# lucidrains/transfusion-pytorch

Measured on NVIDIA H100. Metric: train tokens/sec (text+latent) at d=512 L=8 seq=1024, higher is better.
Workload: dtype bf16

## Files before the change

transfusion_pytorch_b200/csrc/attention_sm90.cu:

```cuda
#include "sm90_ptx.cuh"
#include "common.cuh"
#include "gemm_sm90.cuh"
#include "../../include/tfx_b200.h"

namespace tfx {

int num_sms();

constexpr int FA_BM = 128, FA_BN = 128;
constexpr int FA_THREADS = 256;
constexpr int FA_SMEM = 16384 * 5 + 1024  + 256 ;
constexpr float FA_YMAX = 0.75f;

#define FA_C0 9.9999722832e-01f
#define FA_C1 -3.3323076483e-01f
#define FA_C2 1.3226091649e-01f
#define FA_C3 -4.9280448379e-02f
#define FA_C4 1.2318833231e-02f

__global__ void attn_fast_params_k(const float* __restrict__ gq, const float* __restrict__ gk, int n, float scale, float cap, float* __restrict__ params) {
  const int lane = threadIdx.x;
  float a = 0.f, b = 0.f;
  for (int i = lane; i < n; i += 32) { a = fmaxf(a, fabsf(gq[i] + 1.f)); b = fmaxf(b, fabsf(gk[i] + 1.f)); }
  a = warp_max(a); b = warp_max(b);
  if (lane == 0) {
    const float xmax = 1.01f * (float)n * a * b * scale;
    const float ymax = xmax / cap;
    params[0] = (ymax <= FA_YMAX && isfinite(ymax)) ? 1.f : 0.f;
    params[1] = xmax;
  }
}

__device__ __forceinline__ float ex2_approx(float x) { float y; asm("ex2.approx.ftz.f32 %0, %1;" : "=f"(y) : "f"(x)); return y; }

struct FaPoly {
  float a0, a1, a2, a3, a4;
  __device__ __forceinline__ FaPoly(float scale, float cap) {
    const float k1 = scale / cap, KL = cap * 1.4426950408889634f, k2 = k1 * k1;
    a0 = KL * k1 * FA_C0; a1 = KL * k1 * k2 * FA_C1; a2 = KL * k1 * k2 * k2 * FA_C2; a3 = KL * k1 * k2 * k2 * k2 * FA_C3; a4 = KL * k1 * k2 * k2 * k2 * k2 * FA_C4;
  }
  __device__ __forceinline__ float operator()(float x) const {
    const float X = x * x;
    float g = fmaf(a4, X, a3);
    g = fmaf(g, X, a2);
    g = fmaf(g, X, a1);
    g = fmaf(g, X, a0);
    return x * g;
  }
};

__global__ void __launch_bounds__(FA_THREADS, 2)
attn_fwd_tc_k(const __grid_constant__ CUtensorMap tmQ, const __grid_constant__ CUtensorMap tmK, const __grid_constant__ CUtensorMap tmV,
              const float* __restrict__ gates, int H, const int* __restrict__ kv_limit, const int* __restrict__ tile_q0, const int* __restrict__ tile_qend,
              const int* __restrict__ tile_kv0, const int* __restrict__ tile_kvend, __nv_bfloat16* __restrict__ o, long long ld_o, float* __restrict__ lse,
              int M, float scale, float cap, const float* __restrict__ fast) {
  if (fast[0] == 0.f) return;
  extern __shared__ uint8_t fa_smem_raw[];
  uint8_t* smem = reinterpret_cast<uint8_t*>((reinterpret_cast<uintptr_t>(fa_smem_raw) + 1023) & ~uintptr_t(1023));
  uint8_t* sQ = smem;
  uint8_t* sK = smem + 16384;
  uint8_t* sV = smem + 49152;
  uint64_t* bars = reinterpret_cast<uint64_t*>(smem + 81920);
  uint64_t *q_full = bars, *kv_full = bars + 1;

  const int tile = gridDim.x - 1 - blockIdx.x;
  const int head = blockIdx.y;
  const int tid = threadIdx.x, warp = tid >> 5, lane = tid & 31;
  const int cwg = warp >> 2, w4 = warp & 3, g = lane >> 2, t = lane & 3;
  const int q0 = tile_q0[tile], q_end = tile_qend[tile], kv0 = tile_kv0[tile], kv_end = tile_kvend[tile];
  const int n_kv = (kv_end - kv0 + FA_BN - 1) / FA_BN;

  if (tid == 0) {
    tma_prefetch_desc(&tmQ); tma_prefetch_desc(&tmK); tma_prefetch_desc(&tmV);
    mbar_init(q_full, 1); mbar_init(&kv_full[0], 1); mbar_init(&kv_full[1], 1);
    mbar_fence_init();
  }
  __syncthreads();
  if (tid == 0) {
    mbar_expect_tx(q_full, 16384);
    tma_load_2d(&tmQ, q_full, sQ, head * 64, q0);
    for (int j = 0; j < 2 && j < n_kv; ++j) {
      mbar_expect_tx(&kv_full[j], 32768);
      tma_load_2d(&tmK, &kv_full[j], sK + j * 16384, head * 64, kv0 + j * FA_BN);
      tma_load_2d(&tmV, &kv_full[j], sV + j * 16384, head * 64, kv0 + j * FA_BN);
    }
  }

  const int row_a = q0 + cwg * 64 + w4 * 16 + g, row_b = row_a + 8;
  const int lim_a = row_a < q_end ? kv_limit[row_a] : -1;
  const int lim_b = row_b < q_end ? kv_limit[row_b] : -1;
  const FaPoly poly(scale, cap);
  const float m2 = fast[1] * 1.4426950408889634f;
  float oacc[32];
#pragma unroll
  for (int i = 0; i < 32; ++i) oacc[i] = 0.f;
  float l_a = 0.f, l_b = 0.f;
  const uint32_t aQ = smem_u32(sQ) + cwg * 8192;
  mbar_wait(q_full, 0);

  for (int j = 0; j < n_kv; ++j) {
    const int b = j & 1;
    mbar_wait(&kv_full[b], (j >> 1) & 1);
    const uint32_t aK = smem_u32(sK + b * 16384), aV = smem_u32(sV + b * 16384);
    float s[64];
    wgmma_fence();
#pragma unroll
    for (int k = 0; k < 4; ++k) wgmma_m64n128_ss<0, 0>(s, wgmma_desc_sw128(aQ + k * 32, 16, 1024), wgmma_desc_sw128(aK + k * 32, 16, 1024), k > 0 ? 1u : 0u);
    wgmma_commit();
    wgmma_wait<0>();
    wgmma_reg_fence(s);
    const int key0 = kv0 + j * FA_BN;
    uint32_t pf[8][4];
#pragma unroll
    for (int n8 = 0; n8 < 16; ++n8) {
      const int key = key0 + n8 * 8 + 2 * t;
      float p0 = ex2_approx(poly(s[4 * n8]) - m2), p1 = ex2_approx(poly(s[4 * n8 + 1]) - m2);
      float p2 = ex2_approx(poly(s[4 * n8 + 2]) - m2), p3 = ex2_approx(poly(s[4 * n8 + 3]) - m2);
      p0 = key <= lim_a ? p0 : 0.f; p1 = key + 1 <= lim_a ? p1 : 0.f;
      p2 = key <= lim_b ? p2 : 0.f; p3 = key + 1 <= lim_b ? p3 : 0.f;
      l_a += p0 + p1; l_b += p2 + p3;
      pf[n8 >> 1][(n8 & 1) * 2] = pack_bf16(p0, p1);
      pf[n8 >> 1][(n8 & 1) * 2 + 1] = pack_bf16(p2, p3);
    }
    wgmma_reg_fence(oacc);
    wgmma_fence();
#pragma unroll
    for (int kk = 0; kk < 8; ++kk) wgmma_m64n64_rs<1>(oacc, pf[kk], wgmma_desc_sw128(aV + kk * 2048, 8192, 1024), 1u);
    wgmma_commit();
    wgmma_wait<0>();
    wgmma_reg_fence(oacc);
    __syncthreads();
    if (tid == 0 && j + 2 < n_kv) {
      mbar_expect_tx(&kv_full[b], 32768);
      tma_load_2d(&tmK, &kv_full[b], sK + b * 16384, head * 64, kv0 + (j + 2) * FA_BN);
      tma_load_2d(&tmV, &kv_full[b], sV + b * 16384, head * 64, kv0 + (j + 2) * FA_BN);
    }
  }
  l_a += __shfl_xor_sync(0xffffffffu, l_a, 1); l_a += __shfl_xor_sync(0xffffffffu, l_a, 2);
  l_b += __shfl_xor_sync(0xffffffffu, l_b, 1); l_b += __shfl_xor_sync(0xffffffffu, l_b, 2);
  float ga = l_a > 0.f ? 1.f / l_a : 0.f, gb = l_b > 0.f ? 1.f / l_b : 0.f;
  if (gates) {
    if (row_a < q_end) ga *= 1.f / (1.f + __expf(-gates[(long long)row_a * H + head]));
    if (row_b < q_end) gb *= 1.f / (1.f + __expf(-gates[(long long)row_b * H + head]));
  }
  if (row_a < q_end) {
    __nv_bfloat16* dst = o + (long long)row_a * ld_o + head * 64 + 2 * t;
#pragma unroll
    for (int n8 = 0; n8 < 8; ++n8) *reinterpret_cast<uint32_t*>(dst + n8 * 8) = pack_bf16(oacc[4 * n8] * ga, oacc[4 * n8 + 1] * ga);
    if (t == 0 && lse) lse[(long long)head * M + row_a] = fast[1] + logf(l_a);
  }
  if (row_b < q_end) {
    __nv_bfloat16* dst = o + (long long)row_b * ld_o + head * 64 + 2 * t;
#pragma unroll
    for (int n8 = 0; n8 < 8; ++n8) *reinterpret_cast<uint32_t*>(dst + n8 * 8) = pack_bf16(oacc[4 * n8 + 2] * gb, oacc[4 * n8 + 3] * gb);
    if (t == 0 && lse) lse[(long long)head * M + row_b] = fast[1] + logf(l_b);
  }
}


constexpr int FB_BQ = 64;
constexpr int FB_THREADS = 256;
constexpr int FB_SMEM = 16384 * 2  + 8192 * 4  + 16384  + 1024 + 256;

__global__ void __launch_bounds__(FB_THREADS, 1)
attn_bwd_tc_k(const __grid_constant__ CUtensorMap tmQ, const __grid_constant__ CUtensorMap tmK, const __grid_constant__ CUtensorMap tmV,
              const __grid_constant__ CUtensorMap tmDO,
              const float* __restrict__ lse, const float* __restrict__ dsum, const int* __restrict__ kv_limit,
              const int* __restrict__ kt_kv0, const int* __restrict__ kt_kvend, const int* __restrict__ kt_q0, const int* __restrict__ kt_qend,
              const int* __restrict__ kt_order, float* __restrict__ dq,
              float* __restrict__ dk, __nv_bfloat16* __restrict__ dv, long long ld_dv, int M, int H, float scale, float cap, const float* __restrict__ fast) {
  if (fast[0] == 0.f) return;
  extern __shared__ uint8_t fb_smem_raw[];
  uint8_t* smem = reinterpret_cast<uint8_t*>((reinterpret_cast<uintptr_t>(fb_smem_raw) + 1023) & ~uintptr_t(1023));
  uint8_t* sK = smem;
  uint8_t* sV = smem + 16384;
  uint8_t* sQ = smem + 32768;
  uint8_t* sDO = smem + 49152;
  uint8_t* sDS = smem + 65536;
  uint64_t* bars = reinterpret_cast<uint64_t*>(smem + 81920);
  uint64_t *kv_full = bars, *qdo_full = bars + 1;

  const int idx = blockIdx.x;
  const int tt = idx / H;
  const int tile = kt_order ? kt_order[tt] : tt;
  const int head = idx - tt * H;
  const int kv0 = kt_kv0[tile], kv_end = kt_kvend[tile], q_begin = kt_q0[tile], q_end = kt_qend[tile];
  const int n_q = (q_end - q_begin + FB_BQ - 1) / FB_BQ;
  const int tid = threadIdx.x, warp = tid >> 5, lane = tid & 31;
  const int cwg = warp >> 2, w4 = warp & 3, g = lane >> 2, t = lane & 3;
  const long long HI = (long long)H * 64;

  if (tid == 0) {
    tma_prefetch_desc(&tmQ); tma_prefetch_desc(&tmK); tma_prefetch_desc(&tmV); tma_prefetch_desc(&tmDO);
    mbar_init(kv_full, 1); mbar_init(&qdo_full[0], 1); mbar_init(&qdo_full[1], 1);
    mbar_fence_init();
  }
  __syncthreads();
  if (tid == 0) {
    mbar_expect_tx(kv_full, 32768);
    tma_load_2d(&tmK, kv_full, sK, head * 64, kv0);
    tma_load_2d(&tmV, kv_full, sV, head * 64, kv0);
    for (int i = 0; i < 2 && i < n_q; ++i) {
      mbar_expect_tx(&qdo_full[i], 16384);
      tma_load_2d(&tmQ, &qdo_full[i], sQ + i * 8192, head * 64, q_begin + i * FB_BQ);
      tma_load_2d(&tmDO, &qdo_full[i], sDO + i * 8192, head * 64, q_begin + i * FB_BQ);
    }
  }

  const FaPoly poly(scale, cap);
  const float KL = cap * 1.4426950408889634f;
  const float oms_c = -scale / (KL * KL);
  const int key_a = kv0 + cwg * 64 + w4 * 16 + g, key_b = key_a + 8;
  const float* lse_h = lse + (long long)head * M;
  const float* ds_h = dsum + (long long)head * M;
  float dvacc[32], dkacc[32];
#pragma unroll
  for (int i = 0; i < 32; ++i) { dvacc[i] = 0.f; dkacc[i] = 0.f; }
  const uint32_t aK = smem_u32(sK) + cwg * 8192, aV = smem_u32(sV) + cwg * 8192, aDS = smem_u32(sDS) + cwg * 8192;
  const int ds_row0 = cwg * 64 + w4 * 16 + g;
  mbar_wait(kv_full, 0);

  for (int i = 0; i < n_q; ++i) {
    const int b = i & 1;
    const int qb = q_begin + i * FB_BQ;
    mbar_wait(&qdo_full[b], (i >> 1) & 1);
    const uint32_t aQ = smem_u32(sQ + b * 8192), aDO = smem_u32(sDO + b * 8192);
    float sacc[32], pacc[32];
    wgmma_fence();
#pragma unroll
    for (int k = 0; k < 4; ++k) wgmma_m64n64_ss<0, 0>(sacc, wgmma_desc_sw128(aK + k * 32, 16, 1024), wgmma_desc_sw128(aQ + k * 32, 16, 1024), k > 0 ? 1u : 0u);
#pragma unroll
    for (int k = 0; k < 4; ++k) wgmma_m64n64_ss<0, 0>(pacc, wgmma_desc_sw128(aV + k * 32, 16, 1024), wgmma_desc_sw128(aDO + k * 32, 16, 1024), k > 0 ? 1u : 0u);
    wgmma_commit();
    wgmma_wait<0>();
    wgmma_reg_fence(sacc);
    wgmma_reg_fence(pacc);
    uint32_t pf[4][4], dsf[4][4];
#pragma unroll
    for (int n8 = 0; n8 < 8; ++n8) {
      float pv[4], dsv[4];
#pragma unroll
      for (int c = 0; c < 2; ++c) {
        const int qr = qb + n8 * 8 + 2 * t + c;
        const bool ok = qr < q_end;
        const int lim = ok ? kv_limit[qr] : -1;
        const float lse2 = ok ? lse_h[qr] * 1.4426950408889634f : 0.f;
        const float Dq = ok ? ds_h[qr] : 0.f;
#pragma unroll
        for (int r = 0; r < 2; ++r) {
          const int e = 4 * n8 + 2 * r + c;
          const float e2 = poly(sacc[e]);
          float p = ex2_approx(e2 - lse2);
          p = ((r == 0 ? key_a : key_b) <= lim) ? p : 0.f;
          pv[2 * r + c] = p;
          dsv[2 * r + c] = p * (pacc[e] - Dq) * fmaf(e2 * e2, oms_c, scale);
        }
      }
      pf[n8 >> 1][(n8 & 1) * 2] = pack_bf16(pv[0], pv[1]);
      pf[n8 >> 1][(n8 & 1) * 2 + 1] = pack_bf16(pv[2], pv[3]);
      dsf[n8 >> 1][(n8 & 1) * 2] = pack_bf16(dsv[0], dsv[1]);
      dsf[n8 >> 1][(n8 & 1) * 2 + 1] = pack_bf16(dsv[2], dsv[3]);
    }
    named_bar_sync(1 + cwg, 128);
#pragma unroll
    for (int n8 = 0; n8 < 8; ++n8) {
      const int r0 = ds_row0, r1 = ds_row0 + 8;
      *reinterpret_cast<uint32_t*>(sDS + r0 * 128 + ((n8 ^ (r0 & 7)) << 4) + t * 4) = dsf[n8 >> 1][(n8 & 1) * 2];
      *reinterpret_cast<uint32_t*>(sDS + r1 * 128 + ((n8 ^ (r1 & 7)) << 4) + t * 4) = dsf[n8 >> 1][(n8 & 1) * 2 + 1];
    }
    fence_proxy_async_smem();
    named_bar_sync(1 + cwg, 128);
    float qacc[32];
    wgmma_reg_fence(dvacc);
    wgmma_reg_fence(dkacc);
    wgmma_fence();
#pragma unroll
    for (int kk = 0; kk < 4; ++kk) wgmma_m64n64_rs<1>(dvacc, pf[kk], wgmma_desc_sw128(aDO + kk * 2048, 8192, 1024), 1u);
#pragma unroll
    for (int kk = 0; kk < 4; ++kk) wgmma_m64n64_rs<1>(dkacc, dsf[kk], wgmma_desc_sw128(aQ + kk * 2048, 8192, 1024), 1u);
#pragma unroll
    for (int kk = 0; kk < 4; ++kk) wgmma_m64n64_ss<1, 1>(qacc, wgmma_desc_sw128(aDS + kk * 2048, 8192, 1024), wgmma_desc_sw128(aK + kk * 2048, 8192, 1024), kk > 0 ? 1u : 0u);
    wgmma_commit();
    wgmma_wait<0>();
    wgmma_reg_fence(dvacc);
    wgmma_reg_fence(dkacc);
    wgmma_reg_fence(qacc);
    {
      const int r_a = qb + w4 * 16 + g, r_b = r_a + 8;
#pragma unroll
      for (int n8 = 0; n8 < 8; ++n8) {
        if (r_a < q_end) {
          float* d = dq + (long long)r_a * HI + head * 64 + n8 * 8 + 2 * t;
          asm volatile("red.global.add.v2.f32 [%0], {%1, %2};" ::"l"(d), "f"(qacc[4 * n8]), "f"(qacc[4 * n8 + 1]) : "memory");
        }
        if (r_b < q_end) {
          float* d = dq + (long long)r_b * HI + head * 64 + n8 * 8 + 2 * t;
          asm volatile("red.global.add.v2.f32 [%0], {%1, %2};" ::"l"(d), "f"(qacc[4 * n8 + 2]), "f"(qacc[4 * n8 + 3]) : "memory");
        }
      }
    }
    __syncthreads();
    if (tid == 0 && i + 2 < n_q) {
      mbar_expect_tx(&qdo_full[b], 16384);
      tma_load_2d(&tmQ, &qdo_full[b], sQ + b * 8192, head * 64, q_begin + (i + 2) * FB_BQ);
      tma_load_2d(&tmDO, &qdo_full[b], sDO + b * 8192, head * 64, q_begin + (i + 2) * FB_BQ);
    }
  }
#pragma unroll
  for (int n8 = 0; n8 < 8; ++n8) {
    if (key_a < kv_end) {
      *reinterpret_cast<float2*>(dk + (long long)key_a * HI + head * 64 + n8 * 8 + 2 * t) = make_float2(dkacc[4 * n8], dkacc[4 * n8 + 1]);
      *reinterpret_cast<uint32_t*>(dv + (long long)key_a * ld_dv + head * 64 + n8 * 8 + 2 * t) = pack_bf16(dvacc[4 * n8], dvacc[4 * n8 + 1]);
    }
    if (key_b < kv_end) {
      *reinterpret_cast<float2*>(dk + (long long)key_b * HI + head * 64 + n8 * 8 + 2 * t) = make_float2(dkacc[4 * n8 + 2], dkacc[4 * n8 + 3]);
      *reinterpret_cast<uint32_t*>(dv + (long long)key_b * ld_dv + head * 64 + n8 * 8 + 2 * t) = pack_bf16(dvacc[4 * n8 + 2], dvacc[4 * n8 + 3]);
    }
  }
}

}

using namespace tfx;
#define ST(s) reinterpret_cast<cudaStream_t>(s)

extern "C" {

int tfx_attn_fast_params(const float* q_gamma, const float* k_gamma, int dim_head, float scale, float softcap, float* params, void* stream) {
  TFX_REQUIRE(dim_head > 0 && softcap > 0.f, "attn_fast_params: bad arguments");
  attn_fast_params_k<<<1, 32, 0, ST(stream)>>>(q_gamma, k_gamma, dim_head, scale, softcap, params);
  return check_launch("attn_fast_params");
}

int tfx_attn_fwd_tc(const void* q, const void* k, const void* v, long long ld_q, long long ld_k, long long ld_v, const float* gates, int H,
                    const int* kv_limit, const int* tile_q0, const int* tile_qend, const int* tile_kv0, const int* tile_kvend, int n_tiles,
                    void* o, long long ld_o, float* lse, int M, int M_kv, float scale, float softcap, const float* fast_params, void* stream) {
  if (n_tiles <= 0) return 0;
  if (M_kv <= 0) M_kv = M;
  TFX_REQUIRE(fast_params != nullptr, "attn_fwd_tc: fast_params (from tfx_attn_fast_params) is required");
  TFX_REQUIRE(ld_q % 8 == 0 && ld_k % 8 == 0 && ld_v % 8 == 0 && ld_o % 8 == 0, "attn_fwd_tc: row pitches must be multiples of 8 bf16");
  CUtensorMap tq, tk, tv;
  int rc;
  if ((rc = make_tmap_bf16(&tq, q, (long long)H * 64, M, ld_q, FA_BM)) || (rc = make_tmap_bf16(&tk, k, (long long)H * 64, M_kv, ld_k, FA_BN)) ||
      (rc = make_tmap_bf16(&tv, v, (long long)H * 64, M_kv, ld_v, FA_BN))) {
    set_error("attn_fwd_tc: cuTensorMapEncodeTiled failed (%d)", rc);
    return rc;
  }
  static bool attr_set = false;
  if (!attr_set) {
    if (cudaFuncSetAttribute(attn_fwd_tc_k, cudaFuncAttributeMaxDynamicSharedMemorySize, FA_SMEM) != cudaSuccess) { set_error("attn_fwd_tc: cannot raise dynamic smem"); return -2; }
    attr_set = true;
  }
  attn_fwd_tc_k<<<dim3(n_tiles, H), FA_THREADS, FA_SMEM, ST(stream)>>>(tq, tk, tv, gates, H, kv_limit, tile_q0, tile_qend, tile_kv0, tile_kvend, (__nv_bfloat16*)o, ld_o, lse, M,
                                                                      scale, softcap, fast_params);
  return check_launch("attn_fwd_tc");
}

int tfx_attn_bwd_tc(const void* q, const void* k, const void* v, const void* do_pre, long long ld_q, long long ld_k, long long ld_v, long long ld_do,
                    const float* lse, const float* dsum_hm, const int* kv_limit, const int* kt_kv0, const int* kt_kvend, const int* kt_q0, const int* kt_qend,
                    const int* kt_order, int n_kv_tiles, float* dq, float* dk, void* dv, long long ld_dv, int M, int H, float scale, float softcap, const float* fast_params,
                    void* stream) {
  if (n_kv_tiles <= 0) return 0;
  TFX_REQUIRE(fast_params != nullptr, "attn_bwd_tc: fast_params (from tfx_attn_fast_params) is required");
  TFX_REQUIRE(ld_q % 8 == 0 && ld_k % 8 == 0 && ld_v % 8 == 0 && ld_do % 8 == 0 && ld_dv % 8 == 0, "attn_bwd_tc: row pitches must be multiples of 8 bf16");
  CUtensorMap tq, tk, tv, tdo;
  int rc;
  if ((rc = make_tmap_bf16(&tq, q, (long long)H * 64, M, ld_q, FB_BQ)) || (rc = make_tmap_bf16(&tk, k, (long long)H * 64, M, ld_k, FA_BN)) ||
      (rc = make_tmap_bf16(&tv, v, (long long)H * 64, M, ld_v, FA_BN)) || (rc = make_tmap_bf16(&tdo, do_pre, (long long)H * 64, M, ld_do, FB_BQ))) {
    set_error("attn_bwd_tc: cuTensorMapEncodeTiled failed (%d)", rc);
    return rc;
  }
  static bool attr_set = false;
  if (!attr_set) {
    if (cudaFuncSetAttribute(attn_bwd_tc_k, cudaFuncAttributeMaxDynamicSharedMemorySize, FB_SMEM) != cudaSuccess) { set_error("attn_bwd_tc: cannot raise dynamic smem"); return -2; }
    attr_set = true;
  }
  attn_bwd_tc_k<<<n_kv_tiles * H, FB_THREADS, FB_SMEM, ST(stream)>>>(tq, tk, tv, tdo, lse, dsum_hm, kv_limit, kt_kv0, kt_kvend, kt_q0, kt_qend, kt_order, dq, dk,
                                                                     (__nv_bfloat16*)dv, ld_dv, M, H, scale, softcap, fast_params);
  return check_launch("attn_bwd_tc");
}

}
```

transfusion_pytorch_b200/csrc/sm90_ptx.cuh:

```cuda
#pragma once
#include <cuda.h>
#include <cuda_runtime.h>
#include <cuda_bf16.h>
#include <stdint.h>
#include <stdio.h>

namespace tfx {

#ifndef TFX_SPIN_LIMIT
#define TFX_SPIN_LIMIT (1u << 24)
#endif

__device__ __forceinline__ uint32_t smem_u32(const void* p) {
  return static_cast<uint32_t>(__cvta_generic_to_shared(p));
}

__device__ __forceinline__ void mbar_init(uint64_t* bar, uint32_t count) {
  asm volatile("mbarrier.init.shared::cta.b64 [%0], %1;" ::"r"(smem_u32(bar)), "r"(count));
}
__device__ __forceinline__ void mbar_fence_init() {
  asm volatile("fence.mbarrier_init.release.cluster;" ::: "memory");
}
__device__ __forceinline__ void mbar_expect_tx(uint64_t* bar, uint32_t bytes) {
  asm volatile("mbarrier.arrive.expect_tx.shared::cta.b64 _, [%0], %1;" ::"r"(smem_u32(bar)), "r"(bytes) : "memory");
}
__device__ __forceinline__ void mbar_arrive(uint64_t* bar) {
  asm volatile("mbarrier.arrive.shared::cta.b64 _, [%0];" ::"r"(smem_u32(bar)) : "memory");
}
__device__ __forceinline__ bool mbar_try_wait(uint64_t* bar, uint32_t parity) {
  uint32_t ok;
  asm volatile(
      "{\n\t.reg .pred p;\n\t"
      "mbarrier.try_wait.parity.shared::cta.b64 p, [%1], %2;\n\t"
      "selp.u32 %0, 1, 0, p;\n\t}"
      : "=r"(ok) : "r"(smem_u32(bar)), "r"(parity) : "memory");
  return ok != 0;
}
__device__ __forceinline__ void mbar_wait(uint64_t* bar, uint32_t parity) {
  uint32_t spins = 0;
  while (!mbar_try_wait(bar, parity)) {
    if (++spins > TFX_SPIN_LIMIT) {
#if defined(TFX_DEBUG_SPIN) && TFX_DEBUG_SPIN
      printf("tfx: mbarrier timeout block %d thread %d bar %u parity %u\n", blockIdx.x, threadIdx.x, smem_u32(bar), parity);
#endif
      __trap();
    }
  }
}

__device__ __forceinline__ void tma_prefetch_desc(const CUtensorMap* m) {
  asm volatile("prefetch.tensormap [%0];" ::"l"(reinterpret_cast<uint64_t>(m)) : "memory");
}
__device__ __forceinline__ void tma_load_2d(const CUtensorMap* m, uint64_t* bar, void* smem, int c0, int c1) {
  asm volatile(
      "cp.async.bulk.tensor.2d.shared::cluster.global.mbarrier::complete_tx::bytes [%0], [%1, {%3, %4}], [%2];"
      ::"r"(smem_u32(smem)), "l"(reinterpret_cast<uint64_t>(m)), "r"(smem_u32(bar)), "r"(c0), "r"(c1)
      : "memory");
}
__device__ __forceinline__ void tma_load_2d_multicast(const CUtensorMap* m, uint64_t* bar, void* smem, int c0, int c1, uint16_t mask) {
  asm volatile(
      "cp.async.bulk.tensor.2d.shared::cluster.global.mbarrier::complete_tx::bytes.multicast::cluster [%0], [%1, {%3, %4}], [%2], %5;"
      ::"r"(smem_u32(smem)), "l"(reinterpret_cast<uint64_t>(m)), "r"(smem_u32(bar)), "r"(c0), "r"(c1), "h"(mask)
      : "memory");
}
__device__ __forceinline__ uint32_t cluster_ctarank() { uint32_t r; asm volatile("mov.u32 %0, %%cluster_ctarank;" : "=r"(r)); return r; }
__device__ __forceinline__ void cluster_sync_all() {
  asm volatile("barrier.cluster.arrive.release.aligned;\n\tbarrier.cluster.wait.acquire.aligned;" ::: "memory");
}
__device__ __forceinline__ void mbar_arrive_cluster(uint64_t* bar, uint32_t rank) {
  uint32_t remote;
  asm volatile("mapa.shared::cluster.u32 %0, %1, %2;" : "=r"(remote) : "r"(smem_u32(bar)), "r"(rank));
  asm volatile("mbarrier.arrive.release.cluster.shared::cluster.b64 _, [%0];" ::"r"(remote) : "memory");
}
__device__ __forceinline__ void fence_proxy_async_smem() {
  asm volatile("fence.proxy.async.shared::cta;" ::: "memory");
}
__device__ __forceinline__ void named_bar_sync(int id, int count) {
  asm volatile("bar.sync %0, %1;" ::"r"(id), "r"(count) : "memory");
}
__device__ __forceinline__ void named_bar_arrive(int id, int count) {
  asm volatile("bar.arrive %0, %1;" ::"r"(id), "r"(count) : "memory");
}

template <int N> __device__ __forceinline__ void setmaxnreg_dec() { asm volatile("setmaxnreg.dec.sync.aligned.u32 %0;" ::"n"(N)); }
template <int N> __device__ __forceinline__ void setmaxnreg_inc() { asm volatile("setmaxnreg.inc.sync.aligned.u32 %0;" ::"n"(N)); }

__device__ __forceinline__ void wgmma_fence() { asm volatile("wgmma.fence.sync.aligned;" ::: "memory"); }
__device__ __forceinline__ void wgmma_commit() { asm volatile("wgmma.commit_group.sync.aligned;" ::: "memory"); }
template <int N> __device__ __forceinline__ void wgmma_wait() { asm volatile("wgmma.wait_group.sync.aligned %0;" ::"n"(N) : "memory"); }
template <int N> __device__ __forceinline__ void wgmma_reg_fence(float (&d)[N]) {
#pragma unroll
  for (int i = 0; i < N; ++i) asm volatile("" : "+f"(d[i])::"memory");
}

template <int TA, int TB>
__device__ __forceinline__ void wgmma_m64n128_ss(float (&d)[64], uint64_t da, uint64_t db, uint32_t accumulate) {
  asm volatile(
      "{\n\t.reg .pred p;\n\t"
      "setp.ne.b32 p, %66, 0;\n\t"
      "wgmma.mma_async.sync.aligned.m64n128k16.f32.bf16.bf16 "
      "{%0, %1, %2, %3, %4, %5, %6, %7, %8, %9, %10, %11, %12, %13, %14, %15, %16, %17, %18, %19, %20, %21, %22, %23, %24, %25, %26, %27, %28, %29, %30, %31, %32, %33, %34, %35, %36, %37, %38, %39, %40, %41, %42, %43, %44, %45, %46, %47, %48, %49, %50, %51, %52, %53, %54, %55, %56, %57, %58, %59, %60, %61, %62, %63}, "
      "%64, %65, p, 1, 1, %67, %68;\n\t}"
      : "+f"(d[0]), "+f"(d[1]), "+f"(d[2]), "+f"(d[3]), "+f"(d[4]), "+f"(d[5]), "+f"(d[6]), "+f"(d[7]), "+f"(d[8]), "+f"(d[9]), "+f"(d[10]), "+f"(d[11]), "+f"(d[12]), "+f"(d[13]), "+f"(d[14]), "+f"(d[15]), "+f"(d[16]), "+f"(d[17]), "+f"(d[18]), "+f"(d[19]), "+f"(d[20]), "+f"(d[21]), "+f"(d[22]), "+f"(d[23]), "+f"(d[24]), "+f"(d[25]), "+f"(d[26]), "+f"(d[27]), "+f"(d[28]), "+f"(d[29]), "+f"(d[30]), "+f"(d[31]), "+f"(d[32]), "+f"(d[33]), "+f"(d[34]), "+f"(d[35]), "+f"(d[36]), "+f"(d[37]), "+f"(d[38]), "+f"(d[39]), "+f"(d[40]), "+f"(d[41]), "+f"(d[42]), "+f"(d[43]), "+f"(d[44]), "+f"(d[45]), "+f"(d[46]), "+f"(d[47]), "+f"(d[48]), "+f"(d[49]), "+f"(d[50]), "+f"(d[51]), "+f"(d[52]), "+f"(d[53]), "+f"(d[54]), "+f"(d[55]), "+f"(d[56]), "+f"(d[57]), "+f"(d[58]), "+f"(d[59]), "+f"(d[60]), "+f"(d[61]), "+f"(d[62]), "+f"(d[63])
      : "l"(da), "l"(db), "r"(accumulate), "n"(TA), "n"(TB));
}
template <int TA, int TB>
__device__ __forceinline__ void wgmma_m64n64_ss(float (&d)[32], uint64_t da, uint64_t db, uint32_t accumulate) {
  asm volatile(
      "{\n\t.reg .pred p;\n\t"
      "setp.ne.b32 p, %34, 0;\n\t"
      "wgmma.mma_async.sync.aligned.m64n64k16.f32.bf16.bf16 "
      "{%0, %1, %2, %3, %4, %5, %6, %7, %8, %9, %10, %11, %12, %13, %14, %15, %16, %17, %18, %19, %20, %21, %22, %23, %24, %25, %26, %27, %28, %29, %30, %31}, "
      "%32, %33, p, 1, 1, %35, %36;\n\t}"
      : "+f"(d[0]), "+f"(d[1]), "+f"(d[2]), "+f"(d[3]), "+f"(d[4]), "+f"(d[5]), "+f"(d[6]), "+f"(d[7]), "+f"(d[8]), "+f"(d[9]), "+f"(d[10]), "+f"(d[11]), "+f"(d[12]), "+f"(d[13]), "+f"(d[14]), "+f"(d[15]), "+f"(d[16]), "+f"(d[17]), "+f"(d[18]), "+f"(d[19]), "+f"(d[20]), "+f"(d[21]), "+f"(d[22]), "+f"(d[23]), "+f"(d[24]), "+f"(d[25]), "+f"(d[26]), "+f"(d[27]), "+f"(d[28]), "+f"(d[29]), "+f"(d[30]), "+f"(d[31])
      : "l"(da), "l"(db), "r"(accumulate), "n"(TA), "n"(TB));
}
template <int TB>
__device__ __forceinline__ void wgmma_m64n64_rs(float (&d)[32], const uint32_t (&a)[4], uint64_t db, uint32_t accumulate) {
  asm volatile(
      "{\n\t.reg .pred p;\n\t"
      "setp.ne.b32 p, %37, 0;\n\t"
      "wgmma.mma_async.sync.aligned.m64n64k16.f32.bf16.bf16 "
      "{%0, %1, %2, %3, %4, %5, %6, %7, %8, %9, %10, %11, %12, %13, %14, %15, %16, %17, %18, %19, %20, %21, %22, %23, %24, %25, %26, %27, %28, %29, %30, %31}, "
      "{%32, %33, %34, %35}, %36, p, 1, 1, %38;\n\t}"
      : "+f"(d[0]), "+f"(d[1]), "+f"(d[2]), "+f"(d[3]), "+f"(d[4]), "+f"(d[5]), "+f"(d[6]), "+f"(d[7]), "+f"(d[8]), "+f"(d[9]), "+f"(d[10]), "+f"(d[11]), "+f"(d[12]), "+f"(d[13]), "+f"(d[14]), "+f"(d[15]), "+f"(d[16]), "+f"(d[17]), "+f"(d[18]), "+f"(d[19]), "+f"(d[20]), "+f"(d[21]), "+f"(d[22]), "+f"(d[23]), "+f"(d[24]), "+f"(d[25]), "+f"(d[26]), "+f"(d[27]), "+f"(d[28]), "+f"(d[29]), "+f"(d[30]), "+f"(d[31])
      : "r"(a[0]), "r"(a[1]), "r"(a[2]), "r"(a[3]), "l"(db), "r"(accumulate), "n"(TB));
}

__device__ __forceinline__ uint64_t wgmma_desc_sw128(uint32_t smem_addr, uint32_t lbo_bytes, uint32_t sbo_bytes) {
  uint64_t d = 0;
  d |= (uint64_t)((smem_addr >> 4) & 0x3FFF);
  d |= (uint64_t)((lbo_bytes >> 4) & 0x3FFF) << 16;
  d |= (uint64_t)((sbo_bytes >> 4) & 0x3FFF) << 32;
  d |= (uint64_t)1 << 62;
  return d;
}

}
```

Baseline: 874,600.

## Pipeline attention backward with stage ring, TMA row loads and TMA dQ reduce

The attention backward kernel now uses a four-stage mbarrier ring for Q/dO tiles and brings per-row kv_limit, LSE and D vectors in by 1D TMA instead of scattered global loads. The dQ GEMM alternates between the two warpgroups over full K, through double-buffered dS, and its result is written to swizzled smem and reduced into global memory with TMA reduce-add instead of per-thread red.global atomics. Forward and backward probability computation get unmasked fast paths when a whole tile is visible, and the softcap polynomial subtraction is folded into an fma. The aim is to overlap loads with compute and cut atomic and masking overhead, at the cost of more complex synchronisation and a 16-byte alignment requirement on auxiliary buffers.

```diff
diff --git a/transfusion_pytorch_b200/csrc/attention_sm90.cu b/transfusion_pytorch_b200/csrc/attention_sm90.cu
--- a/transfusion_pytorch_b200/csrc/attention_sm90.cu
+++ b/transfusion_pytorch_b200/csrc/attention_sm90.cu
@@ -39,15 +39,34 @@
     const float k1 = scale / cap, KL = cap * 1.4426950408889634f, k2 = k1 * k1;
     a0 = KL * k1 * FA_C0; a1 = KL * k1 * k2 * FA_C1; a2 = KL * k1 * k2 * k2 * FA_C2; a3 = KL * k1 * k2 * k2 * k2 * FA_C3; a4 = KL * k1 * k2 * k2 * k2 * k2 * FA_C4;
   }
-  __device__ __forceinline__ float operator()(float x) const {
+  __device__ __forceinline__ float operator()(float x) const { return x * tail(x); }
+  __device__ __forceinline__ float minus(float x, float m) const { return fmaf(x, tail(x), -m); }
+  __device__ __forceinline__ float tail(float x) const {
     const float X = x * x;
     float g = fmaf(a4, X, a3);
     g = fmaf(g, X, a2);
     g = fmaf(g, X, a1);
-    g = fmaf(g, X, a0);
-    return x * g;
+    return fmaf(g, X, a0);
   }
 };
+
+template <bool MASKED>
+__device__ __forceinline__ void fwd_p(const float (&s)[64], uint32_t (&pf)[8][4], float& l_a, float& l_b, int key0, int lim_a, int lim_b,
+                                      const FaPoly& poly, float m2, int t) {
+#pragma unroll
+  for (int n8 = 0; n8 < 16; ++n8) {
+    const int key = key0 + n8 * 8 + 2 * t;
+    float p0 = ex2_approx(poly.minus(s[4 * n8], m2)), p1 = ex2_approx(poly.minus(s[4 * n8 + 1], m2));
+    float p2 = ex2_approx(poly.minus(s[4 * n8 + 2], m2)), p3 = ex2_approx(poly.minus(s[4 * n8 + 3], m2));
+    if (MASKED) {
+      p0 = key <= lim_a ? p0 : 0.f; p1 = key + 1 <= lim_a ? p1 : 0.f;
+      p2 = key <= lim_b ? p2 : 0.f; p3 = key + 1 <= lim_b ? p3 : 0.f;
+    }
+    l_a += p0 + p1; l_b += p2 + p3;
+    pf[n8 >> 1][(n8 & 1) * 2] = pack_bf16(p0, p1);
+    pf[n8 >> 1][(n8 & 1) * 2 + 1] = pack_bf16(p2, p3);
+  }
+}
 
 __global__ void __launch_bounds__(FA_THREADS, 2)
 attn_fwd_tc_k(const __grid_constant__ CUtensorMap tmQ, const __grid_constant__ CUtensorMap tmK, const __grid_constant__ CUtensorMap tmV,
@@ -111,17 +130,8 @@
     wgmma_reg_fence(s);
     const int key0 = kv0 + j * FA_BN;
     uint32_t pf[8][4];
-#pragma unroll
-    for (int n8 = 0; n8 < 16; ++n8) {
-      const int key = key0 + n8 * 8 + 2 * t;
-      float p0 = ex2_approx(poly(s[4 * n8]) - m2), p1 = ex2_approx(poly(s[4 * n8 + 1]) - m2);
-      float p2 = ex2_approx(poly(s[4 * n8 + 2]) - m2), p3 = ex2_approx(poly(s[4 * n8 + 3]) - m2);
-      p0 = key <= lim_a ? p0 : 0.f; p1 = key + 1 <= lim_a ? p1 : 0.f;
-      p2 = key <= lim_b ? p2 : 0.f; p3 = key + 1 <= lim_b ? p3 : 0.f;
-      l_a += p0 + p1; l_b += p2 + p3;
-      pf[n8 >> 1][(n8 & 1) * 2] = pack_bf16(p0, p1);
-      pf[n8 >> 1][(n8 & 1) * 2 + 1] = pack_bf16(p2, p3);
-    }
+    if (__all_sync(0xffffffffu, key0 + FA_BN - 1 <= min(lim_a, lim_b))) fwd_p<false>(s, pf, l_a, l_b, key0, lim_a, lim_b, poly, m2, t);
+    else fwd_p<true>(s, pf, l_a, l_b, key0, lim_a, lim_b, poly, m2, t);
     wgmma_reg_fence(oacc);
     wgmma_fence();
 #pragma unroll
@@ -160,25 +170,62 @@
 
 constexpr int FB_BQ = 64;
 constexpr int FB_THREADS = 256;
-constexpr int FB_SMEM = 16384 * 2  + 8192 * 4  + 16384  + 1024 + 256;
+constexpr int FB_STAGES = 4;
+constexpr int FB_STAGE = 16384;
+constexpr int FB_RING = 32768;
+constexpr int FB_ROW_BOX = FB_BQ + 4;
+constexpr int FB_ROW_SLOT = 384, FB_ROWS_STAGE = 3 * FB_ROW_SLOT;
+constexpr int FB_ROWS = FB_RING + FB_STAGES * FB_STAGE;
+constexpr int FB_DS = FB_ROWS + ((FB_STAGES * FB_ROWS_STAGE + 1023) & ~1023);
+constexpr int FB_DQ = FB_DS + 2 * 16384;
+constexpr int FB_BAR = FB_DQ + 2 * 16384;
+constexpr int FB_SMEM = FB_BAR + 256 + 1024 ;
+constexpr int FB_BAR_DS_FULL = 1, FB_BAR_DS_EMPTY = 3, FB_BAR_DQ = 5;
+
+template <bool MASKED>
+__device__ __forceinline__ void bwd_p(float (&sacc)[32], uint32_t (&pf)[4][4], const int* sLim, const float* sLse, int key_a, int key_b, int qvalid,
+                                      const FaPoly& poly, float oms_c, float scale, int t) {
+#pragma unroll
+  for (int n8 = 0; n8 < 8; ++n8) {
+    const int c0 = n8 * 8 + 2 * t;
+    const float lse2[2] = {sLse[c0] * 1.4426950408889634f, sLse[c0 + 1] * 1.4426950408889634f};
+    int lim[2] = {0, 0};
+    if (MASKED) {
+      lim[0] = c0 < qvalid ? sLim[c0] : -1;
+      lim[1] = c0 + 1 < qvalid ? sLim[c0 + 1] : -1;
+    }
+    float pv[4];
+#pragma unroll
+    for (int r = 0; r < 2; ++r)
+#pragma unroll
+      for (int c = 0; c < 2; ++c) {
+        const int e = 4 * n8 + 2 * r + c;
+        const float e2 = poly(sacc[e]);
+        float p = ex2_approx(e2 - lse2[c]);
+        if (MASKED) p = ((r == 0 ? key_a : key_b) <= lim[c]) ? p : 0.f;
+        pv[2 * r + c] = p;
+        sacc[e] = p * fmaf(e2 * e2, oms_c, scale);
+      }
+    pf[n8 >> 1][(n8 & 1) * 2] = pack_bf16(pv[0], pv[1]);
+    pf[n8 >> 1][(n8 & 1) * 2 + 1] = pack_bf16(pv[2], pv[3]);
+  }
+}
 
 __global__ void __launch_bounds__(FB_THREADS, 1)
 attn_bwd_tc_k(const __grid_constant__ CUtensorMap tmQ, const __grid_constant__ CUtensorMap tmK, const __grid_constant__ CUtensorMap tmV,
-              const __grid_constant__ CUtensorMap tmDO,
-              const float* __restrict__ lse, const float* __restrict__ dsum, const int* __restrict__ kv_limit,
+              const __grid_constant__ CUtensorMap tmDO, const __grid_constant__ CUtensorMap tmLim, const __grid_constant__ CUtensorMap tmLse,
+              const __grid_constant__ CUtensorMap tmD, const __grid_constant__ CUtensorMap tmDQ,
               const int* __restrict__ kt_kv0, const int* __restrict__ kt_kvend, const int* __restrict__ kt_q0, const int* __restrict__ kt_qend,
-              const int* __restrict__ kt_order, float* __restrict__ dq,
-              float* __restrict__ dk, __nv_bfloat16* __restrict__ dv, long long ld_dv, int M, int H, float scale, float cap, const float* __restrict__ fast) {
+              const int* __restrict__ kt_order, float* __restrict__ dk, __nv_bfloat16* __restrict__ dv, long long ld_dv, int M, int H, float scale, float cap,
+              const float* __restrict__ fast) {
   if (fast[0] == 0.f) return;
   extern __shared__ uint8_t fb_smem_raw[];
   uint8_t* smem = reinterpret_cast<uint8_t*>((reinterpret_cast<uintptr_t>(fb_smem_raw) + 1023) & ~uintptr_t(1023));
   uint8_t* sK = smem;
   uint8_t* sV = smem + 16384;
-  uint8_t* sQ = smem + 32768;
-  uint8_t* sDO = smem + 49152;
-  uint8_t* sDS = smem + 65536;
-  uint64_t* bars = reinterpret_cast<uint64_t*>(smem + 81920);
-  uint64_t *kv_full = bars, *qdo_full = bars + 1;
+  uint8_t* sDS = smem + FB_DS;
+  uint64_t* bars = reinterpret_cast<uint64_t*>(smem + FB_BAR);
+  uint64_t *full = bars, *empty = bars + FB_STAGES, *kv_full = bars + 2 * FB_STAGES;
 
   const int idx = blockIdx.x;
   const int tt = idx / H;
@@ -187,90 +234,95 @@
   const int kv0 = kt_kv0[tile], kv_end = kt_kvend[tile], q_begin = kt_q0[tile], q_end = kt_qend[tile];
   const int n_q = (q_end - q_begin + FB_BQ - 1) / FB_BQ;
   const int tid = threadIdx.x, warp = tid >> 5, lane = tid & 31;
-  const int cwg = warp >> 2, w4 = warp & 3, g = lane >> 2, t = lane & 3;
-  const long long HI = (long long)H * 64;
 
   if (tid == 0) {
     tma_prefetch_desc(&tmQ); tma_prefetch_desc(&tmK); tma_prefetch_desc(&tmV); tma_prefetch_desc(&tmDO);
-    mbar_init(kv_full, 1); mbar_init(&qdo_full[0], 1); mbar_init(&qdo_full[1], 1);
+    for (int s = 0; s < FB_STAGES; ++s) { mbar_init(&full[s], 1); mbar_init(&empty[s], 8); }
+    mbar_init(kv_full, 1);
     mbar_fence_init();
   }
   __syncthreads();
+
+  auto load_step = [&](int j) {
+    const int sl = j % FB_STAGES;
+    const int qb = q_begin + j * FB_BQ;
+    uint8_t* st = smem + FB_RING + sl * FB_STAGE;
+    uint8_t* rows = smem + FB_ROWS + sl * FB_ROWS_STAGE;
+    mbar_expect_tx(&full[sl], FB_STAGE + 3 * FB_ROW_BOX * 4);
+    tma_load_2d(&tmQ, &full[sl], st, head * 64, qb);
+    tma_load_2d(&tmDO, &full[sl], st + 8192, head * 64, qb);
+    tma_load_1d(&tmLim, &full[sl], rows, qb & ~3);
+    tma_load_1d(&tmLse, &full[sl], rows + FB_ROW_SLOT, (head * M + qb) & ~3);
+    tma_load_1d(&tmD, &full[sl], rows + 2 * FB_ROW_SLOT, (head * M + qb) & ~3);
+  };
   if (tid == 0) {
     mbar_expect_tx(kv_full, 32768);
     tma_load_2d(&tmK, kv_full, sK, head * 64, kv0);
     tma_load_2d(&tmV, kv_full, sV, head * 64, kv0);
-    for (int i = 0; i < 2 && i < n_q; ++i) {
-      mbar_expect_tx(&qdo_full[i], 16384);
-      tma_load_2d(&tmQ, &qdo_full[i], sQ + i * 8192, head * 64, q_begin + i * FB_BQ);
-      tma_load_2d(&tmDO, &qdo_full[i], sDO + i * 8192, head * 64, q_begin + i * FB_BQ);
-    }
-  }
-
+    for (int j = 0; j < FB_STAGES && j < n_q; ++j) load_step(j);
+  }
+  const int cwg = warp >> 2, w4 = warp & 3, g = lane >> 2, t = lane & 3;
+  const bool leader = (tid & 127) == 0;
   const FaPoly poly(scale, cap);
   const float KL = cap * 1.4426950408889634f;
   const float oms_c = -scale / (KL * KL);
   const int key_a = kv0 + cwg * 64 + w4 * 16 + g, key_b = key_a + 8;
-  const float* lse_h = lse + (long long)head * M;
-  const float* ds_h = dsum + (long long)head * M;
+  const int warp_key_last = kv0 + cwg * 64 + w4 * 16 + 15;
   float dvacc[32], dkacc[32];
 #pragma unroll
   for (int i = 0; i < 32; ++i) { dvacc[i] = 0.f; dkacc[i] = 0.f; }
-  const uint32_t aK = smem_u32(sK) + cwg * 8192, aV = smem_u32(sV) + cwg * 8192, aDS = smem_u32(sDS) + cwg * 8192;
+  const uint32_t aK = smem_u32(sK) + cwg * 8192, aV = smem_u32(sV) + cwg * 8192, aKall = smem_u32(sK);
   const int ds_row0 = cwg * 64 + w4 * 16 + g;
+  uint8_t* sDQ = smem + FB_DQ + cwg * 16384;
   mbar_wait(kv_full, 0);
 
+  int s = 0; uint32_t phase = 0;
   for (int i = 0; i < n_q; ++i) {
     const int b = i & 1;
     const int qb = q_begin + i * FB_BQ;
-    mbar_wait(&qdo_full[b], (i >> 1) & 1);
-    const uint32_t aQ = smem_u32(sQ + b * 8192), aDO = smem_u32(sDO + b * 8192);
+    mbar_wait(&full[s], phase);
+    const uint32_t aQ = smem_u32(smem + FB_RING + s * FB_STAGE), aDO = aQ + 8192;
+    const int* sLim = reinterpret_cast<const int*>(smem + FB_ROWS + s * FB_ROWS_STAGE) + (qb & 3);
+    const float* sLse = reinterpret_cast<const float*>(smem + FB_ROWS + s * FB_ROWS_STAGE + FB_ROW_SLOT) + ((head * M + qb) & 3);
+    const float* sD = reinterpret_cast<const float*>(smem + FB_ROWS + s * FB_ROWS_STAGE + 2 * FB_ROW_SLOT) + ((head * M + qb) & 3);
     float sacc[32], pacc[32];
     wgmma_fence();
 #pragma unroll
     for (int k = 0; k < 4; ++k) wgmma_m64n64_ss<0, 0>(sacc, wgmma_desc_sw128(aK + k * 32, 16, 1024), wgmma_desc_sw128(aQ + k * 32, 16, 1024), k > 0 ? 1u : 0u);
+    wgmma_commit();
 #pragma unroll
     for (int k = 0; k < 4; ++k) wgmma_m64n64_ss<0, 0>(pacc, wgmma_desc_sw128(aV + k * 32, 16, 1024), wgmma_desc_sw128(aDO + k * 32, 16, 1024), k > 0 ? 1u : 0u);
     wgmma_commit();
+    if (tid == 0 && i >= 2 && i - 2 + FB_STAGES < n_q) {
+      mbar_wait(&empty[(i - 2) % FB_STAGES], ((i - 2) / FB_STAGES) & 1);
+      load_step(i - 2 + FB_STAGES);
+    }
+    const int qvalid = q_end - qb;
+    const bool full_vis = qvalid >= FB_BQ && warp_key_last <= __reduce_min_sync(0xffffffffu, min(sLim[lane], sLim[lane + 32]));
+    wgmma_wait<1>();
+    wgmma_reg_fence(sacc);
+    uint32_t pf[4][4], dsf[4][4];
+    if (full_vis) bwd_p<false>(sacc, pf, sLim, sLse, key_a, key_b, qvalid, poly, oms_c, scale, t);
+    else bwd_p<true>(sacc, pf, sLim, sLse, key_a, key_b, qvalid, poly, oms_c, scale, t);
     wgmma_wait<0>();
-    wgmma_reg_fence(sacc);
     wgmma_reg_fence(pacc);
-    uint32_t pf[4][4], dsf[4][4];
 #pragma unroll
     for (int n8 = 0; n8 < 8; ++n8) {
-      float pv[4], dsv[4];
-#pragma unroll
-      for (int c = 0; c < 2; ++c) {
-        const int qr = qb + n8 * 8 + 2 * t + c;
-        const bool ok = qr < q_end;
-        const int lim = ok ? kv_limit[qr] : -1;
-        const float lse2 = ok ? lse_h[qr] * 1.4426950408889634f : 0.f;
-        const float Dq = ok ? ds_h[qr] : 0.f;
-#pragma unroll
-        for (int r = 0; r < 2; ++r) {
-          const int e = 4 * n8 + 2 * r + c;
-          const float e2 = poly(sacc[e]);
-          float p = ex2_approx(e2 - lse2);
-          p = ((r == 0 ? key_a : key_b) <= lim) ? p : 0.f;
-          pv[2 * r + c] = p;
-          dsv[2 * r + c] = p * (pacc[e] - Dq) * fmaf(e2 * e2, oms_c, scale);
-        }
-      }
-      pf[n8 >> 1][(n8 & 1) * 2] = pack_bf16(pv[0], pv[1]);
-      pf[n8 >> 1][(n8 & 1) * 2 + 1] = pack_bf16(pv[2], pv[3]);
-      dsf[n8 >> 1][(n8 & 1) * 2] = pack_bf16(dsv[0], dsv[1]);
-      dsf[n8 >> 1][(n8 & 1) * 2 + 1] = pack_bf16(dsv[2], dsv[3]);
-    }
-    named_bar_sync(1 + cwg, 128);
+      const float d0 = sD[n8 * 8 + 2 * t], d1 = sD[n8 * 8 + 2 * t + 1];
+      dsf[n8 >> 1][(n8 & 1) * 2] = pack_bf16(sacc[4 * n8] * (pacc[4 * n8] - d0), sacc[4 * n8 + 1] * (pacc[4 * n8 + 1] - d1));
+      dsf[n8 >> 1][(n8 & 1) * 2 + 1] = pack_bf16(sacc[4 * n8 + 2] * (pacc[4 * n8 + 2] - d0), sacc[4 * n8 + 3] * (pacc[4 * n8 + 3] - d1));
+    }
+    uint8_t* dsb = sDS + b * 16384;
+    if (cwg != b && i >= 2) named_bar_sync(FB_BAR_DS_EMPTY + b, 256);
 #pragma unroll
     for (int n8 = 0; n8 < 8; ++n8) {
       const int r0 = ds_row0, r1 = ds_row0 + 8;
-      *reinterpret_cast<uint32_t*>(sDS + r0 * 128 + ((n8 ^ (r0 & 7)) << 4) + t * 4) = dsf[n8 >> 1][(n8 & 1) * 2];
-      *reinterpret_cast<uint32_t*>(sDS + r1 * 128 + ((n8 ^ (r1 & 7)) << 4) + t * 4) = dsf[n8 >> 1][(n8 & 1) * 2 + 1];
+      *reinterpret_cast<uint32_t*>(dsb + r0 * 128 + ((n8 ^ (r0 & 7)) << 4) + t * 4) = dsf[n8 >> 1][(n8 & 1) * 2];
+      *reinterpret_cast<uint32_t*>(dsb + r1 * 128 + ((n8 ^ (r1 & 7)) << 4) + t * 4) = dsf[n8 >> 1][(n8 & 1) * 2 + 1];
     }
     fence_proxy_async_smem();
-    named_bar_sync(1 + cwg, 128);
-    float qacc[32];
+    if (cwg == b) named_bar_sync(FB_BAR_DS_FULL + b, 256);
+    else named_bar_arrive(FB_BAR_DS_FULL + b, 256);
     wgmma_reg_fence(dvacc);
     wgmma_reg_fence(dkacc);
     wgmma_fence();
@@ -278,45 +330,80 @@
     for (int kk = 0; kk < 4; ++kk) wgmma_m64n64_rs<1>(dvacc, pf[kk], wgmma_desc_sw128(aDO + kk * 2048, 8192, 1024), 1u);
 #pragma unroll
     for (int kk = 0; kk < 4; ++kk) wgmma_m64n64_rs<1>(dkacc, dsf[kk], wgmma_desc_sw128(aQ + kk * 2048, 8192, 1024), 1u);
-#pragma unroll
-    for (int kk = 0; kk < 4; ++kk) wgmma_m64n64_ss<1, 1>(qacc, wgmma_desc_sw128(aDS + kk * 2048, 8192, 1024), wgmma_desc_sw128(aK + kk * 2048, 8192, 1024), kk > 0 ? 1u : 0u);
     wgmma_commit();
-    wgmma_wait<0>();
-    wgmma_reg_fence(dvacc);
-    wgmma_reg_fence(dkacc);
-    wgmma_reg_fence(qacc);
-    {
-      const int r_a = qb + w4 * 16 + g, r_b = r_a + 8;
+    if (cwg == b) {
+      float qacc[32];
+      const uint32_t aDS = smem_u32(dsb);
+      wgmma_fence();
+#pragma unroll
+      for (int kk = 0; kk < 8; ++kk) wgmma_m64n64_ss<1, 1>(qacc, wgmma_desc_sw128(aDS + kk * 2048, 8192, 1024), wgmma_desc_sw128(aKall + kk * 2048, 8192, 1024), kk > 0 ? 1u : 0u);
+      wgmma_commit();
+      wgmma_wait<0>();
+      wgmma_reg_fence(dvacc);
+      wgmma_reg_fence(dkacc);
+      wgmma_reg_fence(qacc);
+      __syncwarp();
+      if (lane == 0) mbar_arrive(&empty[s]);
+      if (i + 2 < n_q) named_bar_arrive(FB_BAR_DS_EMPTY + b, 256);
+      if (leader) bulk_wait_read_all();
+      named_bar_sync(FB_BAR_DQ + cwg, 128);
+      const int r0 = w4 * 16 + g, r1 = r0 + 8;
 #pragma unroll
       for (int n8 = 0; n8 < 8; ++n8) {
-        if (r_a < q_end) {
-          float* d = dq + (long long)r_a * HI + head * 64 + n8 * 8 + 2 * t;
-          asm volatile("red.global.add.v2.f32 [%0], {%1, %2};" ::"l"(d), "f"(qacc[4 * n8]), "f"(qacc[4 * n8 + 1]) : "memory");
-        }
-        if (r_b < q_end) {
-          float* d = dq + (long long)r_b * HI + head * 64 + n8 * 8 + 2 * t;
-          asm volatile("red.global.add.v2.f32 [%0], {%1, %2};" ::"l"(d), "f"(qacc[4 * n8 + 2]), "f"(qacc[4 * n8 + 3]) : "memory");
-        }
+        const int chunk = 2 * (n8 & 3) + (t >> 1), off = (n8 >> 2) * 8192 + (t & 1) * 8;
+        *reinterpret_cast<float2*>(sDQ + off + r0 * 128 + ((chunk ^ (r0 & 7)) << 4)) = make_float2(qacc[4 * n8], qacc[4 * n8 + 1]);
+        *reinterpret_cast<float2*>(sDQ + off + r1 * 128 + ((chunk ^ (r1 & 7)) << 4)) = make_float2(qacc[4 * n8 + 2], qacc[4 * n8 + 3]);
       }
-    }
-    __syncthreads();
-    if (tid == 0 && i + 2 < n_q) {
-      mbar_expect_tx(&qdo_full[b], 16384);
-      tma_load_2d(&tmQ, &qdo_full[b], sQ + b * 8192, head * 64, q_begin + (i + 2) * FB_BQ);
-      tma_load_2d(&tmDO, &qdo_full[b], sDO + b * 8192, head * 64, q_begin + (i + 2) * FB_BQ);
-    }
-  }
+      fence_proxy_async_smem();
+      named_bar_sync(FB_BAR_DQ + cwg, 128);
+      if (leader) {
+        tma_reduce_add_2d(&tmDQ, sDQ, head * 64, qb);
+        tma_reduce_add_2d(&tmDQ, sDQ + 8192, head * 64 + 32, qb);
+        bulk_commit();
+      }
+    } else {
+      wgmma_wait<0>();
+      wgmma_reg_fence(dvacc);
+      wgmma_reg_fence(dkacc);
+      __syncwarp();
+      if (lane == 0) mbar_arrive(&empty[s]);
+    }
+    if (++s == FB_STAGES) { s = 0; phase ^= 1; }
+  }
+  if (leader) bulk_wait_all();
 #pragma unroll
   for (int n8 = 0; n8 < 8; ++n8) {
     if (key_a < kv_end) {
-      *reinterpret_cast<float2*>(dk + (long long)key_a * HI + head * 64 + n8 * 8 + 2 * t) = make_float2(dkacc[4 * n8], dkacc[4 * n8 + 1]);
+      *reinterpret_cast<float2*>(dk + (long long)key_a * H * 64 + head * 64 + n8 * 8 + 2 * t) = make_float2(dkacc[4 * n8], dkacc[4 * n8 + 1]);
       *reinterpret_cast<uint32_t*>(dv + (long long)key_a * ld_dv + head * 64 + n8 * 8 + 2 * t) = pack_bf16(dvacc[4 * n8], dvacc[4 * n8 + 1]);
     }
     if (key_b < kv_end) {
-      *reinterpret_cast<float2*>(dk + (long long)key_b * HI + head * 64 + n8 * 8 + 2 * t) = make_float2(dkacc[4 * n8 + 2], dkacc[4 * n8 + 3]);
+      *reinterpret_cast<float2*>(dk + (long long)key_b * H * 64 + head * 64 + n8 * 8 + 2 * t) = make_float2(dkacc[4 * n8 + 2], dkacc[4 * n8 + 3]);
       *reinterpret_cast<uint32_t*>(dv + (long long)key_b * ld_dv + head * 64 + n8 * 8 + 2 * t) = pack_bf16(dvacc[4 * n8 + 2], dvacc[4 * n8 + 3]);
     }
   }
+}
+
+inline int make_tmap_rows(CUtensorMap* tm, CUtensorMapDataType type, const void* ptr, long long n) {
+  PFN_encodeTiled enc = get_encode_fn();
+  if (!enc) return -1;
+  cuuint64_t dims[1] = {(cuuint64_t)n};
+  cuuint64_t strides[1] = {0};
+  cuuint32_t box[1] = {FB_ROW_BOX}, estr[1] = {1};
+  CUresult r = enc(tm, type, 1, const_cast<void*>(ptr), dims, strides, box, estr, CU_TENSOR_MAP_INTERLEAVE_NONE, CU_TENSOR_MAP_SWIZZLE_NONE,
+                   CU_TENSOR_MAP_L2_PROMOTION_NONE, CU_TENSOR_MAP_FLOAT_OOB_FILL_NONE);
+  return r == CUDA_SUCCESS ? 0 : -(int)r - 1000;
+}
+
+inline int make_tmap_dq(CUtensorMap* tm, float* dq, int M, int H) {
+  PFN_encodeTiled enc = get_encode_fn();
+  if (!enc) return -1;
+  cuuint64_t dims[2] = {(cuuint64_t)H * 64, (cuuint64_t)M};
+  cuuint64_t strides[1] = {(cuuint64_t)H * 64 * 4};
+  cuuint32_t box[2] = {32, FB_BQ}, estr[2] = {1, 1};
+  CUresult r = enc(tm, CU_TENSOR_MAP_DATA_TYPE_FLOAT32, 2, dq, dims, strides, box, estr, CU_TENSOR_MAP_INTERLEAVE_NONE, CU_TENSOR_MAP_SWIZZLE_128B,
+                   CU_TENSOR_MAP_L2_PROMOTION_L2_256B, CU_TENSOR_MAP_FLOAT_OOB_FILL_NONE);
+  return r == CUDA_SUCCESS ? 0 : -(int)r - 1000;
 }
 
 }
@@ -363,11 +450,13 @@
   if (n_kv_tiles <= 0) return 0;
   TFX_REQUIRE(fast_params != nullptr, "attn_bwd_tc: fast_params (from tfx_attn_fast_params) is required");
   TFX_REQUIRE(ld_q % 8 == 0 && ld_k % 8 == 0 && ld_v % 8 == 0 && ld_do % 8 == 0 && ld_dv % 8 == 0, "attn_bwd_tc: row pitches must be multiples of 8 bf16");
-  CUtensorMap tq, tk, tv, tdo;
+  CUtensorMap tq, tk, tv, tdo, tlim, tlse, td, tdq;
   int rc;
   if ((rc = make_tmap_bf16(&tq, q, (long long)H * 64, M, ld_q, FB_BQ)) || (rc = make_tmap_bf16(&tk, k, (long long)H * 64, M, ld_k, FA_BN)) ||
-      (rc = make_tmap_bf16(&tv, v, (long long)H * 64, M, ld_v, FA_BN)) || (rc = make_tmap_bf16(&tdo, do_pre, (long long)H * 64, M, ld_do, FB_BQ))) {
-    set_error("attn_bwd_tc: cuTensorMapEncodeTiled failed (%d)", rc);
+      (rc = make_tmap_bf16(&tv, v, (long long)H * 64, M, ld_v, FA_BN)) || (rc = make_tmap_bf16(&tdo, do_pre, (long long)H * 64, M, ld_do, FB_BQ)) ||
+      (rc = make_tmap_rows(&tlim, CU_TENSOR_MAP_DATA_TYPE_INT32, kv_limit, M)) || (rc = make_tmap_rows(&tlse, CU_TENSOR_MAP_DATA_TYPE_FLOAT32, lse, (long long)H * M)) ||
+      (rc = make_tmap_rows(&td, CU_TENSOR_MAP_DATA_TYPE_FLOAT32, dsum_hm, (long long)H * M)) || (rc = make_tmap_dq(&tdq, dq, M, H))) {
+    set_error("attn_bwd_tc: cuTensorMapEncodeTiled failed (%d): kv_limit, lse, dsum and dq must be 16-byte aligned", rc);
     return rc;
   }
   static bool attr_set = false;
@@ -375,7 +464,7 @@
     if (cudaFuncSetAttribute(attn_bwd_tc_k, cudaFuncAttributeMaxDynamicSharedMemorySize, FB_SMEM) != cudaSuccess) { set_error("attn_bwd_tc: cannot raise dynamic smem"); return -2; }
     attr_set = true;
   }
-  attn_bwd_tc_k<<<n_kv_tiles * H, FB_THREADS, FB_SMEM, ST(stream)>>>(tq, tk, tv, tdo, lse, dsum_hm, kv_limit, kt_kv0, kt_kvend, kt_q0, kt_qend, kt_order, dq, dk,
+  attn_bwd_tc_k<<<n_kv_tiles * H, FB_THREADS, FB_SMEM, ST(stream)>>>(tq, tk, tv, tdo, tlim, tlse, td, tdq, kt_kv0, kt_kvend, kt_q0, kt_qend, kt_order, dk,
                                                                      (__nv_bfloat16*)dv, ld_dv, M, H, scale, softcap, fast_params);
   return check_launch("attn_bwd_tc");
 }
diff --git a/transfusion_pytorch_b200/csrc/sm90_ptx.cuh b/transfusion_pytorch_b200/csrc/sm90_ptx.cuh
--- a/transfusion_pytorch_b200/csrc/sm90_ptx.cuh
+++ b/transfusion_pytorch_b200/csrc/sm90_ptx.cuh
@@ -57,6 +57,19 @@
       ::"r"(smem_u32(smem)), "l"(reinterpret_cast<uint64_t>(m)), "r"(smem_u32(bar)), "r"(c0), "r"(c1)
       : "memory");
 }
+__device__ __forceinline__ void tma_load_1d(const CUtensorMap* m, uint64_t* bar, void* smem, int c0) {
+  asm volatile(
+      "cp.async.bulk.tensor.1d.shared::cluster.global.mbarrier::complete_tx::bytes [%0], [%1, {%3}], [%2];"
+      ::"r"(smem_u32(smem)), "l"(reinterpret_cast<uint64_t>(m)), "r"(smem_u32(bar)), "r"(c0)
+      : "memory");
+}
+__device__ __forceinline__ void tma_reduce_add_2d(const CUtensorMap* m, const void* smem, int c0, int c1) {
+  asm volatile("cp.reduce.async.bulk.tensor.2d.global.shared::cta.add.tile.bulk_group [%0, {%2, %3}], [%1];"
+               ::"l"(reinterpret_cast<uint64_t>(m)), "r"(smem_u32(smem)), "r"(c0), "r"(c1) : "memory");
+}
+__device__ __forceinline__ void bulk_commit() { asm volatile("cp.async.bulk.commit_group;" ::: "memory"); }
+__device__ __forceinline__ void bulk_wait_read_all() { asm volatile("cp.async.bulk.wait_group.read 0;" ::: "memory"); }
+__device__ __forceinline__ void bulk_wait_all() { asm volatile("cp.async.bulk.wait_group 0;" ::: "memory"); }
 __device__ __forceinline__ void tma_load_2d_multicast(const CUtensorMap* m, uint64_t* bar, void* smem, int c0, int c1, uint16_t mask) {
   asm volatile(
       "cp.async.bulk.tensor.2d.shared::cluster.global.mbarrier::complete_tx::bytes.multicast::cluster [%0], [%1, {%3, %4}], [%2], %5;"
```

Measured after the change: 935,500, median of 6. 7.0% higher.
